# theovincent/iS-DQN

Hardware: AMD Instinct MI355X
Metric: gradient-steps/sec (batch=256, K=9, 84x84x4) (higher is better)
Workload: dtype bf16x3 (split-bf16 MFMA operands hi+lo, fp32 accumulate)

## Files before the change

### is-dqn_amd/csrc/conv_u8_pair.h

```cpp
#pragma once
#include "conv_img.h"

namespace isdqn {

constexpr int U8P_PB = 2;

template <int PASSES, int NSTEPS>
__global__ __launch_bounds__(GEMM_THREADS, 4) void conv_fwd_u8_pair_kernel(const ConvImgParams p) {
    ISDQN_EMPTY_KERNEL_RETURN
    constexpr int MT = 2, NT = 2, MTW = MT, NTHR = GEMM_THREADS, STACK_MAX = 4;
    using T = ConvImgTraits<MT, PASSES, true>;
    using GA = typename T::GA;
    extern __shared__ __attribute__((aligned(16))) char smem_raw[];
    __bf16* smem = reinterpret_cast<__bf16*>(smem_raw);
    __bf16* a_stage = smem;
    __bf16* img = smem + 2 * T::A_STAGE;
    const ConvGeom& g = p.g;
    const int tid = threadIdx.x, lane = tid & 63, wave = tid >> 6, grp = lane >> 4;
#if defined(ISDQN_DEV)
#define U8P_STAMP(i)                                                                                 \
    if (p.stamps != nullptr && threadIdx.x == 0) {                                                  \
        p.stamps[(int64_t)blockIdx.x * 8 + (i)] = (long long)__builtin_amdgcn_s_memtime();           \
        if ((i) == 0) p.stamps[(int64_t)blockIdx.x * 8 + 7] = (long long)__builtin_amdgcn_s_memrealtime(); \
    }
#else
#define U8P_STAMP(i)
#endif
    U8P_STAMP(0);
    const int T2 = p.tiles_per_img >> 1;
    int j, tp;
    xcd_image_tile((int)blockIdx.x, p.n_img, T2, j, tp);

    __shared__ __attribute__((aligned(16))) float s_par[3][64];
    float par_v = 0.f;
    {
        const int which = tid >> 6, ch = tid & 63;
        const float* src = which == 0 ? p.bias : which == 1 ? p.gamma : p.beta;
        const bool ok = tid < 192 && ch < g.cout_p && src != nullptr;
        ISDQN_BOUNDS_CHECK(ok ? src + ch : zero_chunk(), 4, 13);
        par_v = *(const ISDQN_GLOBAL float*)(ok ? src + ch : zero_chunk());
    }
    constexpr int nsteps = NSTEPS;
    const int k_last = g.K - 8;
    constexpr int A_PER = (GA::CHUNKS + NTHR - 1) / NTHR;
    int a_row[A_PER], a_var[A_PER], a_lds[A_PER];
    bool a_on[A_PER];
#pragma unroll
    for (int i = 0; i < A_PER; ++i) {
        int c = tid + i * NTHR;
        a_on[i] = c < GA::CHUNKS;
        if (!a_on[i]) c = 0;
        a_row[i] = stash_row(c);
        a_var[i] = (c & 3) * 8;
        a_lds[i] = a_row[i] * GA::PITCH + (c & 3) * 8;
    }
    constexpr int PF = 4;
    float sa[PF][A_PER][8];
    auto fetch = [&](int slot, int k) {
#pragma unroll
        for (int i = 0; i < A_PER; ++i) p.W.load(a_row[i], k + a_var[i], sa[slot][i]);
    };
    auto stash = [&](int slot, int stage) {
        __bf16* a_hi = a_stage + stage * T::A_STAGE;
        __bf16* a_lo = a_hi + GA::ELEMS;
#pragma unroll
        for (int i = 0; i < A_PER; ++i) {
            if (GA::CHUNKS % NTHR != 0 && !a_on[i]) continue;
            bf16x8 hi, lo;
            if constexpr (PASSES >= 2) {
                s8_unpack(sa[slot][i], hi, lo);
                *reinterpret_cast<bf16x8*>(a_lo + a_lds[i]) = lo;
            } else {
                s8_unpack_hi(sa[slot][i], hi);
            }
            *reinterpret_cast<bf16x8*>(a_hi + a_lds[i]) = hi;
        }
    };
    static_assert(NSTEPS >= PF + 2 && NSTEPS % 2 == 0, "ring of four slices + two staged ones");

    const FrameSrc& fs = p.fs;
    const uint8_t* base[STACK_MAX];
#pragma unroll
    for (int c = 0; c < STACK_MAX; ++c) {
        const int id = c < fs.stack ? fs.frame_id(j, c) : -1;
        base[c] = id >= 0 ? fs.frames + (int64_t)id * fs.stride : nullptr;
    }
    const uint8_t* zeros = reinterpret_cast<const uint8_t*>(zero_chunk());
    const int cpr = p.Wp / 8, per_plane = p.R * cpr, plane = p.R * p.Wp;
    unsigned long long raw[U8P_PB][STACK_MAX];
    auto request = [&](int row_base) {
#pragma unroll
        for (int k = 0; k < U8P_PB; ++k) {
            const int pos = k * NTHR + tid;
            const bool on = pos < per_plane;
            uint32_t lr, cx;
            p.d_chunk.divmod((uint32_t)(on ? pos : 0), lr, cx);
            const int iy = row_base + (int)lr, ix0 = (int)cx * 8 - g.pad;
            const bool ok = on && iy >= 0 && iy < fs.H && ix0 > -8 && ix0 < fs.W;
            const int ixc = min(max(ix0, 0), fs.W - 8);
            const int off = iy * fs.W + ixc;
#pragma unroll
            for (int c = 0; c < STACK_MAX; ++c) raw[k][c] = load_u64_unaligned((ok && base[c] != nullptr) ? base[c] + off : zeros);
        }
    };
    auto commit = [&]() {
#pragma unroll
        for (int k = 0; k < U8P_PB; ++k) {
            const int pos = k * NTHR + tid;
            const bool on = pos < per_plane;
            uint32_t lr, cx;
            p.d_chunk.divmod((uint32_t)(on ? pos : 0), lr, cx);
            const int ix0 = (int)cx * 8 - g.pad;
            const int sh = ix0 - min(max(ix0, 0), fs.W - 8);
            const int dst = (int)lr * p.Wp + (int)cx * 8;
#pragma unroll
            for (int c = 0; c < STACK_MAX; ++c) {
                if (c >= fs.stack) continue;
                float v[8];
                FrameSrc::patch8_cvt(raw[k][c], sh, v);
                bf16x8 hi;
                round8(v, hi);
                if (on) *reinterpret_cast<bf16x8*>(img + c * plane + dst) = hi;
            }
        }
    };
    auto tile_rows = [&](int tile) {
        const int oy_min = (int)g.d_wout.div((uint32_t)(tile * 128));
        return oy_min * g.stride - g.pad;
    };

    struct Frags {
        bf16x8 a_hi[MTW], a_lo[MTW], b_hi[NT];
    };

    auto do_tile = [&](auto it_c) {
        constexpr int it = decltype(it_c)::value;
        const int tile = 2 * tp + it;
        const int p0 = tile * 128;
        const int row_base = tile_rows(tile);
        const int full = (p.n_img / 8) * 8;
        const int old_wg8 = j < full ? (j >> 3) * p.tiles_per_img + tile : (j * p.tiles_per_img + tile) >> 3;
        const int rot = (int)((unsigned)old_wg8 % (unsigned)nsteps);
        auto slice = [&](int s) {
            const int k = s + rot;
            return k >= nsteps ? k - nsteps : k;
        };
#pragma unroll
        for (int d = 0; d < PF; ++d) fetch(d, slice(d) * GEMM_BK);
        if constexpr (it == 0) request(row_base);
        commit();
        U8P_STAMP(it == 0 ? 1 : 4);

        int b_org[NT], out_pix[NT];
#pragma unroll
        for (int nt = 0; nt < NT; ++nt) {
            int pp = p0 + wave * 32 + nt * 16 + (lane & 15);
            const bool in_img = pp < g.npix;
            pp = in_img ? pp : g.npix - 1;
            uint32_t oy_u, ox_u;
            g.d_wout.divmod((uint32_t)pp, oy_u, ox_u);
            const int oy = (int)oy_u, ox = (int)ox_u;
            out_pix[nt] = in_img ? oy * g.wout + ox : -1;
            const int ly0 = oy * g.stride - g.pad - row_base;
            const int lx0 = ox * g.stride;
            b_org[nt] = ly0 * p.Wp + lx0;
        }
        f32x4 acc[MTW][NT];
#pragma unroll
        for (int mt = 0; mt < MTW; ++mt)
#pragma unroll
            for (int nt = 0; nt < NT; ++nt) mfma_init(acc[mt][nt]);

        auto read_frags = [&](int stage, int kk, Frags& f) {
            const __bf16* a_hi = a_stage + stage * T::A_STAGE;
            const __bf16* a_lo = a_hi + GA::ELEMS;
#pragma unroll
            for (int mt = 0; mt < MTW; ++mt) {
                f.a_hi[mt] = read_frag<false, GA::PITCH>(a_hi, mt * 16, lane);
                if constexpr (PASSES >= 2) f.a_lo[mt] = read_frag<false, GA::PITCH>(a_lo, mt * 16, lane);
            }
            int kq = kk * GEMM_BK + grp * 8;
            kq = kq < k_last ? kq : k_last;
            const int c = kq >> 6, ky = (kq >> 3) & 7;
            const int tap_off = (c * p.R + ky) * p.Wp;
#pragma unroll
            for (int nt = 0; nt < NT; ++nt) {
                const __bf16* src = img + b_org[nt] + tap_off;
                typedef __attribute__((ext_vector_type(4))) __bf16 bf16x4;
                bf16x4 h0 = *reinterpret_cast<const bf16x4*>(src);
                bf16x4 h1 = *reinterpret_cast<const bf16x4*>(src + 4);
                f.b_hi[nt] = __builtin_shufflevector(h0, h1, 0, 1, 2, 3, 4, 5, 6, 7);
            }
        };
        auto mfma_step = [&](const Frags& f) {
#pragma unroll
            for (int nt = 0; nt < NT; ++nt)
#pragma unroll
                for (int mt = 0; mt < MTW; ++mt) {
                    if constexpr (PASSES >= 2) mfma_acc(acc[mt][nt], f.a_lo[mt], f.b_hi[nt]);
                    mfma_acc(acc[mt][nt], f.a_hi[mt], f.b_hi[nt]);
                }
        };
        Frags fr[2];
        if constexpr (it == 0) {
            if (tid < 192) s_par[tid >> 6][tid & 63] = par_v;
        }
        stash(0, 0);
        stash(1, 1);
        fetch(0, slice(PF) * GEMM_BK);
        fetch(1, slice(PF + 1) * GEMM_BK);
        __syncthreads();
        read_frags(0, slice(0), fr[0]);
        __syncthreads();
#pragma unroll
        for (int s = 0; s < NSTEPS; ++s) {
            if (s + 1 < NSTEPS) read_frags((s + 1) & 1, slice(s + 1), fr[(s + 1) & 1]);
            mfma_step(fr[s & 1]);
            if (s + 2 < NSTEPS) stash((s + 2) % PF, s & 1);
            if (s + 2 + PF < NSTEPS) fetch((s + 2) % PF, slice(s + 2 + PF) * GEMM_BK);
            if constexpr (it == 0) {
                if (s == NSTEPS - 3) request(tile_rows(tile + 1));
            }
            constexpr int N_MFMA = MTW * NT * (PASSES >= 3 ? 3 : PASSES);
#pragma unroll
            for (int i = 0; i < N_MFMA; ++i) {
                __builtin_amdgcn_sched_group_barrier(0x008, 1, 0);
                if (i < N_MFMA / 2) __builtin_amdgcn_sched_group_barrier(0x100, 1, 0);
                __builtin_amdgcn_sched_group_barrier(0x002, 2, 0);
            }
            __syncthreads();
        }

        U8P_STAMP(it == 0 ? 2 : 5);
        float bi[MTW][4], ga[MTW][4], be[MTW][4];
#pragma unroll
        for (int mt = 0; mt < MTW; ++mt) {
            const int ch0 = (mt * 16 + grp * 4) & 63;
            const float4 b4 = *reinterpret_cast<const float4*>(&s_par[0][ch0]);
            const float4 g4 = *reinterpret_cast<const float4*>(&s_par[1][ch0]);
            const float4 e4 = *reinterpret_cast<const float4*>(&s_par[2][ch0]);
            bi[mt][0] = b4.x; bi[mt][1] = b4.y; bi[mt][2] = b4.z; bi[mt][3] = b4.w;
            ga[mt][0] = g4.x; ga[mt][1] = g4.y; ga[mt][2] = g4.z; ga[mt][3] = g4.w;
            be[mt][0] = e4.x; be[mt][1] = e4.y; be[mt][2] = e4.z; be[mt][3] = e4.w;
        }
        const float inv_c = 1.0f / (float)g.cout;
        float zv[NT][MTW][4], s1[NT], s2[NT];
#pragma unroll
        for (int nt = 0; nt < NT; ++nt) {
            s1[nt] = s2[nt] = 0.f;
#pragma unroll
            for (int mt = 0; mt < MTW; ++mt)
#pragma unroll
                for (int r = 0; r < 4; ++r) {
                    int ch = mt * 16 + grp * 4 + r;
                    float zz = ch < g.cout ? acc[mt][nt][r] * p.scale + bi[mt][r] : 0.f;
                    zv[nt][mt][r] = zz;
                    s1[nt] += zz;
                    s2[nt] += zz * zz;
                }
            if (p.gamma != nullptr) {
                s1[nt] += __shfl_xor(s1[nt], 16); s1[nt] += __shfl_xor(s1[nt], 32);
                s2[nt] += __shfl_xor(s2[nt], 16); s2[nt] += __shfl_xor(s2[nt], 32);
            }
        }
#pragma unroll
        for (int nt = 0; nt < NT; ++nt) {
            float mean = 0.f, rstd = 1.f;
            if (p.gamma != nullptr) {
                mean = s1[nt] * inv_c;
                float var = fmaxf(s2[nt] * inv_c - mean * mean, 0.f);
                rstd = rsqrtf(var + 1e-6f);
            }
            if (out_pix[nt] >= 0) {
                const int64_t pix = (int64_t)j * g.npix + out_pix[nt];
#pragma unroll
                for (int mt = 0; mt < MTW; ++mt) {
                    int ch0 = mt * 16 + grp * 4;
                    if (ch0 >= g.cout_p) continue;
                    float4 a, zq;
                    float* ap = &a.x;
                    float* zp = &zq.x;
#pragma unroll
                    for (int r = 0; r < 4; ++r) {
                        float y = p.gamma != nullptr ? (zv[nt][mt][r] - mean) * (rstd * ga[mt][r]) + be[mt][r] : zv[nt][mt][r];
                        ap[r] = (ch0 + r < g.cout) ? fmaxf(y, 0.f) : 0.f;
                        zp[r] = zv[nt][mt][r];
                    }
                    s8_store_quad_paired(p.act + pix * g.cout_p, ch0, a.x, a.y, a.z, a.w);
                    if (j < p.z_img) *reinterpret_cast<float4*>(p.z + pix * g.cout_p + ch0) = zq;
                }
            }
        }
        U8P_STAMP(it == 0 ? 3 : 6);
    };
    do_tile(std::integral_constant<int, 0>{});
    do_tile(std::integral_constant<int, 1>{});
#undef U8P_STAMP
}

template <int PASSES, int NSTEPS>
static int launch_conv_fwd_u8_pair(const ConvImgParams& p, hipStream_t st) {
    using T = ConvImgTraits<2, PASSES, true>;
    const int lds = (2 * T::A_STAGE + T::B_PLANES * p.plane_elems) * 2;
    static LdsConfigured configured;
    if (int rc = ensure_dynamic_lds(&conv_fwd_u8_pair_kernel<PASSES, NSTEPS>, lds, configured)) return rc;
    const int grid = p.n_img * (p.tiles_per_img / 2);
    ISDQN_REPORT_OCCUPANCY((&conv_fwd_u8_pair_kernel<PASSES, NSTEPS>), GEMM_THREADS, lds, grid);
    hipLaunchKernelGGL((conv_fwd_u8_pair_kernel<PASSES, NSTEPS>), dim3(grid), dim3(GEMM_THREADS), lds, st, p);
    ISDQN_HIP_CHECK(hipGetLastError());
    return ISDQN_OK;
}

}
```

### is-dqn_amd/csrc/net_kernels.hip

```cpp
#include <stdarg.h>
#include <stdlib.h>

#include <algorithm>
#include <type_traits>
#include <vector>
#include <atomic>
#include <functional>

#include "conv_img.h"
#include "conv_u8_pair.h"
#include "conv_s8_pair.h"
#include "hl_gauss.h"
#include "net_plan.h"
#include "net_problems.h"

namespace isdqn {

__device__ inline double pow_int(double b, int t) {
    double r = 1.0, x = b;
    for (unsigned u = (unsigned)t; u != 0; u >>= 1) {
        if (u & 1u) r *= x;
        x *= x;
    }
    return r;
}


__global__ __launch_bounds__(256) void dense_post_kernel(const float* __restrict__ slabs, int n_slabs,
                                                         int64_t slab_stride, int64_t row_pitch, int rows, int F, int Fp,
                                                         const float* __restrict__ bias,
                                                         const float* __restrict__ gamma,
                                                         const float* __restrict__ beta, int has_relu,
                                                         float* __restrict__ act, float* __restrict__ z, int z_rows, int act_s8) {
    extern __shared__ float s_row[];
    __shared__ float s_red[2][4];
    const int row = blockIdx.x, tid = threadIdx.x;
    float* s_g = s_row + Fp;
    float* s_b = s_row + 2 * Fp;
    float s1 = 0.f, s2 = 0.f;
    for (int c = 2 * tid; c < Fp; c += 512) {
        float par[3][2];
#pragma unroll
        for (int w = 0; w < 3; ++w) {
            const float* src = w == 0 ? bias : w == 1 ? gamma : beta;
#pragma unroll
            for (int e = 0; e < 2; ++e)
            {
                ISDQN_BOUNDS_CHECK((src != nullptr && c + e < F) ? src + c + e : zero_chunk(), 4, 28);
                par[w][e] = *(const ISDQN_GLOBAL float*)((src != nullptr && c + e < F) ? src + c + e : zero_chunk());
            }
        }
        float v0 = 0.f, v1 = 0.f;
        const float* p = slabs + (int64_t)row * row_pitch + c;
        int s = 0;
        for (; s + 16 <= n_slabs; s += 16) {
            float2 t[16];
#pragma unroll
            for (int u = 0; u < 16; ++u) t[u] = *reinterpret_cast<const float2*>(p + (int64_t)(s + u) * slab_stride);
#pragma unroll
            for (int u = 0; u < 16; ++u) { v0 += t[u].x; v1 += t[u].y; }
        }
        if (s < n_slabs) {
            float2 t[16];
#pragma unroll
            for (int u = 0; u < 16; ++u)
                t[u] = *reinterpret_cast<const float2*>(p + (int64_t)min(s + u, n_slabs - 1) * slab_stride);
#pragma unroll
            for (int u = 0; u < 16; ++u) { v0 += (s + u < n_slabs) ? t[u].x : 0.f; v1 += (s + u < n_slabs) ? t[u].y : 0.f; }
        }
        v0 = c < F ? v0 + par[0][0] : 0.f;
        v1 = c + 1 < F ? v1 + par[0][1] : 0.f;
        s_row[c] = v0;
        s_row[c + 1] = v1;
        s_g[c] = par[1][0]; s_g[c + 1] = par[1][1];
        s_b[c] = par[2][0]; s_b[c + 1] = par[2][1];
        s1 += v0 + v1;
        s2 += v0 * v0 + v1 * v1;
    }
    float mean = 0.f, rstd = 1.f;
    if (gamma != nullptr) {
        for (int off = 32; off > 0; off >>= 1) {
            s1 += __shfl_xor(s1, off);
            s2 += __shfl_xor(s2, off);
        }
        if ((tid & 63) == 0) {
            s_red[0][tid >> 6] = s1;
            s_red[1][tid >> 6] = s2;
        }
        __syncthreads();
        s1 = s_red[0][0] + s_red[0][1] + s_red[0][2] + s_red[0][3];
        s2 = s_red[1][0] + s_red[1][1] + s_red[1][2] + s_red[1][3];
        mean = s1 / (float)F;
        float var = fmaxf(s2 / (float)F - mean * mean, 0.f);
// ... 987 lines not shown
    ConvGeom g;
    g.hin = l.hin; g.win = l.win; g.cin_p = l.cin_p; g.hout = l.hout; g.wout = l.wout;
    g.cout = l.cout; g.cout_p = l.cout_p; g.ksz = l.ksz; g.stride = l.stride; g.pad = l.pad;
    g.npix = l.npix; g.K = l.K;
    g.stride_sh = l.stride == 4 ? 2 : l.stride == 2 ? 1 : 0;
    g.d_npix = FastDiv(l.npix); g.d_wout = FastDiv(l.wout); g.d_cinp = FastDiv(l.cin_p);
    g.d_ksz = FastDiv(l.ksz); g.d_coutp = FastDiv(l.cout_p);
    return g;
}

constexpr int DZ_S8 = 1;

struct NetInput {
    const uint8_t* frames; int64_t frame_stride; const int* frame_ids; int paired_B;
    const float* obs; const float* obs2; int obs_split;
    int id_pitch = 0, id_off = 0;
};

template <int BM, int PASSES, bool U8>
static int launch_conv_fwd(const Layer& l, const float* params, const float* wmir, const NetInput& in, const float* act_in, int n_img,
                           int z_img, float* act, float* z, hipStream_t st) {
    ConvFwd<BM, PASSES, U8> p;
    p.g = conv_geom(l);
    p.W = MatSrc{wmir + l.w_off, l.K, l.cout_p, l.K, 1};
    p.in = act_in;
    p.fs = FrameSrc{in.frames, in.frame_stride, in.frame_ids, l.cin, in.paired_B, l.hin, l.win, in.id_pitch, in.id_off};
    p.bias = params + l.b_off;
    p.gamma = l.has_ln ? params + l.g_off : nullptr;
    p.beta = l.has_ln ? params + l.be_off : nullptr;
    p.scale = U8 ? (1.0f / 255.0f) : 1.0f;
    p.act = act; p.z = z;
    p.n_pix_total = n_img * l.npix;
    p.z_pix = z_img * l.npix;
    return launch_gemm(p, ceil_div(p.n_pix_total, 128), st);
}

static int conv_fwd_img(const Layer& l, bool x3, const float* params, const float* wmir, const NetInput& in, const float* act_in, int n_img,
                        int z_img, float* act, float* z, hipStream_t st, bool* done) {
    *done = false;
    if (act == nullptr || (z == nullptr && z_img > 0)) return ISDQN_OK;
    ConvImgParams ip;
    ip.g = conv_geom(l);
    const int mt = l.cout_p <= 32 ? 2 : 4;
    const int passes = x3 ? (l.is_u8 ? 2 : 3) : 1;
    ip.PP = l.is_u8 ? 0 : l.cin_p + (l.cin_p % 64 == 0 ? 16 : 8);
    int lds = conv_img_geometry(ip.g, l.is_u8, l.cin, passes >= 3 ? 2 : 1, mt, passes >= 2 ? 2 : 1, ip.R, ip.Wp,
                                ip.plane_elems, ip.PP);
    constexpr int LDS_LIMIT = 158 * 1024;
    if (lds > LDS_LIMIT || (l.is_u8 && (l.win < 8 || l.cin > 4))) return ISDQN_OK;
    if (!l.is_u8 && l.cin_p < 16) return ISDQN_OK;
    if (!l.is_u8 && l.npix <= 128) {
        const int want = ip.Wp + (((l.wout - ip.Wp) % 8) + 8) % 8;
        const int planes = passes >= 3 ? 2 : 1;
        const int lds2 = lds + planes * ip.R * (want - ip.Wp) * ip.PP * 2;
        const int stage2 = (passes >= 2 ? 2 : 1) * (mt * 16) * 48 * 2 * 2;
        const int old_total = lds > 80 * 1024 ? lds + stage2 : lds, new_total = lds2 > 80 * 1024 ? lds2 + stage2 : lds2;
        if (want != ip.Wp && new_total <= LDS_LIMIT && (old_total <= 80 * 1024) == (new_total <= 80 * 1024)) {
            ip.Wp = want;
            ip.plane_elems = ip.R * want * ip.PP;
            lds = lds2;
        }
    }
    ip.W = MatSrc{wmir + l.w_off, l.K, l.cout_p, l.K, 1};
    ip.in = act_in;
    ip.fs = FrameSrc{in.frames, in.frame_stride, in.frame_ids, l.cin, in.paired_B, l.hin, l.win, in.id_pitch, in.id_off};
    ip.bias = params + l.b_off;
    ip.gamma = l.has_ln ? params + l.g_off : nullptr;
    ip.beta = l.has_ln ? params + l.be_off : nullptr;
    ip.scale = l.is_u8 ? (1.0f / 255.0f) : 1.0f;
    ip.act = act; ip.z = z; ip.n_img = n_img; ip.z_img = z_img;
    ip.tiles_per_img = ceil_div(l.npix, 128);
    ip.d_chunk = FastDiv((uint32_t)(l.is_u8 ? ip.Wp / 8 : l.cin_p / 8));
    ip.d_Wp = FastDiv((uint32_t)ip.Wp);
    ip.d_R = FastDiv((uint32_t)ip.R);
    ip.order = PixelOrder(l.hout, l.wout, !l.is_u8 && ip.tiles_per_img == 1);
    ip.stamps = stamps_for(l.name);
    ip.ablate = 0;
#if defined(ISDQN_DEV)
    if (const char* e = getenv("ISDQN_ABLATE")) ip.ablate = atoi(e);
#endif
    *done = true;
    if (l.is_u8) {
#if !defined(ISDQN_NO_U8_PAIR)
        if (mt == 2 && ip.tiles_per_img % 2 == 0 && ip.R * (ip.Wp / 8) <= U8P_PB * GEMM_THREADS && l.cin == 4 && l.K == 256 && ip.ablate == 0)
            return passes == 2 ? launch_conv_fwd_u8_pair<2, 8>(ip, st) : launch_conv_fwd_u8_pair<1, 8>(ip, st);
#endif
        if (passes == 2) return mt == 2 ? launch_conv_fwd_img<2, 2, true>(ip, st) : launch_conv_fwd_img<4, 2, true>(ip, st);
        return mt == 2 ? launch_conv_fwd_img<2, 1, true>(ip, st) : launch_conv_fwd_img<4, 1, true>(ip, st);
    }
    const int stage_bytes = (passes >= 2 ? 2 : 1) * (mt * 16) * 48 * 2 * 2;
    static const bool no_kg = ISDQN_DEV_ENV("ISDQN_NO_KGROUPS");
    const bool kg2 = !no_kg && mt == 4 && lds > 80 * 1024 && lds + stage_bytes <= LDS_LIMIT &&
                     mt * 16 * 128 * 4 <= lds - stage_bytes && l.K >= 8 * GEMM_BK;
#if !defined(ISDQN_NO_U8_PAIR)
    if (passes == 3 && mt == 4 && kg2 && ip.tiles_per_img == 1 && l.K == 512 && n_img % 2 == 0 && ip.ablate == 0 && ip.stamps == nullptr &&
        ip.R * ip.Wp * (l.cin_p / 8) <= S8P_BATCH * GEMM_THREADS * 2)
        return launch_conv_fwd_s8_pair<8>(ip, st);
#endif
    if (passes == 3) return mt == 2 ? launch_conv_fwd_img<2, 3, false>(ip, st)
                          : kg2 ? launch_conv_fwd_img<4, 3, false, 2>(ip, st) : launch_conv_fwd_img<4, 3, false>(ip, st);
    return mt == 2 ? launch_conv_fwd_img<2, 1, false>(ip, st)
         : kg2 ? launch_conv_fwd_img<4, 1, false, 2>(ip, st) : launch_conv_fwd_img<4, 1, false>(ip, st);
}

static int conv_fwd(const Layer& l, bool x3, const float* params, const float* wmir, const NetInput& in, const float* act_in, int n_img,
                    int z_img, float* act, float* z, hipStream_t st) {
    bool done = false;
    int rc = conv_fwd_img(l, x3, params, wmir, in, act_in, n_img, z_img, act, z, st, &done);
    if (rc || done) return rc;
    const bool small = l.cout_p <= 32;
    if (l.is_u8) {
        if (x3) return small ? launch_conv_fwd<32, 2, true>(l, params, wmir, in, act_in, n_img, z_img, act, z, st)
                             : launch_conv_fwd<64, 2, true>(l, params, wmir, in, act_in, n_img, z_img, act, z, st);
        return small ? launch_conv_fwd<32, 1, true>(l, params, wmir, in, act_in, n_img, z_img, act, z, st)
                     : launch_conv_fwd<64, 1, true>(l, params, wmir, in, act_in, n_img, z_img, act, z, st);
    }
    if (x3) return small ? launch_conv_fwd<32, 3, false>(l, params, wmir, in, act_in, n_img, z_img, act, z, st)
                         : launch_conv_fwd<64, 3, false>(l, params, wmir, in, act_in, n_img, z_img, act, z, st);
    return small ? launch_conv_fwd<32, 1, false>(l, params, wmir, in, act_in, n_img, z_img, act, z, st)
                 : launch_conv_fwd<64, 1, false>(l, params, wmir, in, act_in, n_img, z_img, act, z, st);
}

template <int BM, int BN, int WM, int WN, bool ATR, bool BTR, int PASSES, bool AL, bool A2PART, bool ADAM = false, int S8M = 0>
static int launch_plain(const MatSrc& A, const float* A2, int a_split, const MatSrc& B, float* C, int ldc, int M,
                        int N, int K, int splits, int64_t slab_stride, hipStream_t st,
                        const AdamFuse* adam = nullptr) {
    PlainGemm<BM, BN, WM, WN, ATR, BTR, PASSES, AL, A2PART, ADAM, S8M> p;
    if (adam) p.adam = *adam;
    p.A = A; p.B = B; p.A2 = A2; p.a_split = a_split; p.C = C; p.ldc = ldc; p.M = M; p.N = N; p.K = K;
    p.tiles_m = ceil_div(M, BM); p.tiles_n = ceil_div(N, BN);
    int ksteps = ceil_div(K, GEMM_BK);
    if (splits < 1) splits = 1;
    if (splits > ksteps) splits = ksteps;
    p.steps_per_split = ceil_div(ksteps, splits);
    p.splits = ceil_div(ksteps, p.steps_per_split);
    p.slab_stride = slab_stride;
    return launch_gemm(p, p.tiles_m * p.tiles_n * p.splits, st);
}
static int effective_splits(int K, int splits) {
    int ksteps = ceil_div(K, GEMM_BK);
    if (splits < 1) splits = 1;
    if (splits > ksteps) splits = ksteps;
    int sps = ceil_div(ksteps, splits);
    return ceil_div(ksteps, sps);
}

template <bool ATR, bool BTR, bool AL = true, bool A2PART = false, int S8M = 0>
static int plain_big(bool x3, const MatSrc& A, const float* A2, int a_split, const MatSrc& B, float* C, int ldc,
                     int M, int N, int K, int splits, int64_t slab_stride, hipStream_t st) {
    if (x3)
        return launch_plain<128, 128, 2, 2, ATR, BTR, 3, AL, A2PART, false, S8M>(A, A2, a_split, B, C, ldc, M, N, K, splits,
                                                                                 slab_stride, st);
    return launch_plain<128, 128, 2, 2, ATR, BTR, 1, AL, A2PART, false, S8M>(A, A2, a_split, B, C, ldc, M, N, K, splits,
                                                                             slab_stride, st);
}

template <bool ATR, bool BTR, int S8M = 0>
static int plain_narrow(bool x3, const MatSrc& A, const MatSrc& B, float* C, int ldc, int M, int N, int K, int splits,
                        int64_t slab_stride, hipStream_t st) {
    if (x3) return launch_plain<128, 64, 2, 2, ATR, BTR, 3, true, false, false, S8M>(A, nullptr, 0, B, C, ldc, M, N, K, splits, slab_stride, st);
    return launch_plain<128, 64, 2, 2, ATR, BTR, 1, true, false, false, S8M>(A, nullptr, 0, B, C, ldc, M, N, K, splits, slab_stride, st);
}

static int dense_fwd(const Layer& l, bool x3, const float* params, const float* wmir, const NetInput& in, const float* act_in, int rows,
                     int z_rows, float* slab, float* act, float* z, hipStream_t st, bool skip_post = false) {
    MatSrc A, B;
    const float* A2 = nullptr;
    int a_split = 0;
// ... 1172 lines not shown
```

Baseline: 4172.

## Replace paired u8 conv kernel with persistent kernel keeping weights resident in LDS

Swaps the two-tile-per-block u8 first-layer conv for a persistent kernel with a grid sized to the CU count. Each workgroup loads the full 32xK weight slab into LDS once and then loops over many image tiles, prefetching the next item's frames while the current one computes. This removes the per-tile weight refetch, the staged-slice ring and the per-step barriers. In exchange it uses more LDS per block, allows only 2 workgroups per CU, and relies on the persistent loop hiding frame-load latency.

```diff
diff --git a/is-dqn_amd/csrc/conv_u8_pair.h b/is-dqn_amd/csrc/conv_u8_pair.h
--- a/is-dqn_amd/csrc/conv_u8_pair.h
+++ /dev/null
@@ -1,314 +0,0 @@
-#pragma once
-#include "conv_img.h"
-
-namespace isdqn {
-
-constexpr int U8P_PB = 2;
-
-template <int PASSES, int NSTEPS>
-__global__ __launch_bounds__(GEMM_THREADS, 4) void conv_fwd_u8_pair_kernel(const ConvImgParams p) {
-    ISDQN_EMPTY_KERNEL_RETURN
-    constexpr int MT = 2, NT = 2, MTW = MT, NTHR = GEMM_THREADS, STACK_MAX = 4;
-    using T = ConvImgTraits<MT, PASSES, true>;
-    using GA = typename T::GA;
-    extern __shared__ __attribute__((aligned(16))) char smem_raw[];
-    __bf16* smem = reinterpret_cast<__bf16*>(smem_raw);
-    __bf16* a_stage = smem;
-    __bf16* img = smem + 2 * T::A_STAGE;
-    const ConvGeom& g = p.g;
-    const int tid = threadIdx.x, lane = tid & 63, wave = tid >> 6, grp = lane >> 4;
-#if defined(ISDQN_DEV)
-#define U8P_STAMP(i)                                                                                 \
-    if (p.stamps != nullptr && threadIdx.x == 0) {                                                  \
-        p.stamps[(int64_t)blockIdx.x * 8 + (i)] = (long long)__builtin_amdgcn_s_memtime();           \
-        if ((i) == 0) p.stamps[(int64_t)blockIdx.x * 8 + 7] = (long long)__builtin_amdgcn_s_memrealtime(); \
-    }
-#else
-#define U8P_STAMP(i)
-#endif
-    U8P_STAMP(0);
-    const int T2 = p.tiles_per_img >> 1;
-    int j, tp;
-    xcd_image_tile((int)blockIdx.x, p.n_img, T2, j, tp);
-
-    __shared__ __attribute__((aligned(16))) float s_par[3][64];
-    float par_v = 0.f;
-    {
-        const int which = tid >> 6, ch = tid & 63;
-        const float* src = which == 0 ? p.bias : which == 1 ? p.gamma : p.beta;
-        const bool ok = tid < 192 && ch < g.cout_p && src != nullptr;
-        ISDQN_BOUNDS_CHECK(ok ? src + ch : zero_chunk(), 4, 13);
-        par_v = *(const ISDQN_GLOBAL float*)(ok ? src + ch : zero_chunk());
-    }
-    constexpr int nsteps = NSTEPS;
-    const int k_last = g.K - 8;
-    constexpr int A_PER = (GA::CHUNKS + NTHR - 1) / NTHR;
-    int a_row[A_PER], a_var[A_PER], a_lds[A_PER];
-    bool a_on[A_PER];
-#pragma unroll
-    for (int i = 0; i < A_PER; ++i) {
-        int c = tid + i * NTHR;
-        a_on[i] = c < GA::CHUNKS;
-        if (!a_on[i]) c = 0;
-        a_row[i] = stash_row(c);
-        a_var[i] = (c & 3) * 8;
-        a_lds[i] = a_row[i] * GA::PITCH + (c & 3) * 8;
-    }
-    constexpr int PF = 4;
-    float sa[PF][A_PER][8];
-    auto fetch = [&](int slot, int k) {
-#pragma unroll
-        for (int i = 0; i < A_PER; ++i) p.W.load(a_row[i], k + a_var[i], sa[slot][i]);
-    };
-    auto stash = [&](int slot, int stage) {
-        __bf16* a_hi = a_stage + stage * T::A_STAGE;
-        __bf16* a_lo = a_hi + GA::ELEMS;
-#pragma unroll
-        for (int i = 0; i < A_PER; ++i) {
-            if (GA::CHUNKS % NTHR != 0 && !a_on[i]) continue;
-            bf16x8 hi, lo;
-            if constexpr (PASSES >= 2) {
-                s8_unpack(sa[slot][i], hi, lo);
-                *reinterpret_cast<bf16x8*>(a_lo + a_lds[i]) = lo;
-            } else {
-                s8_unpack_hi(sa[slot][i], hi);
-            }
-            *reinterpret_cast<bf16x8*>(a_hi + a_lds[i]) = hi;
-        }
-    };
-    static_assert(NSTEPS >= PF + 2 && NSTEPS % 2 == 0, "ring of four slices + two staged ones");
-
-    const FrameSrc& fs = p.fs;
-    const uint8_t* base[STACK_MAX];
-#pragma unroll
-    for (int c = 0; c < STACK_MAX; ++c) {
-        const int id = c < fs.stack ? fs.frame_id(j, c) : -1;
-        base[c] = id >= 0 ? fs.frames + (int64_t)id * fs.stride : nullptr;
-    }
-    const uint8_t* zeros = reinterpret_cast<const uint8_t*>(zero_chunk());
-    const int cpr = p.Wp / 8, per_plane = p.R * cpr, plane = p.R * p.Wp;
-    unsigned long long raw[U8P_PB][STACK_MAX];
-    auto request = [&](int row_base) {
-#pragma unroll
-        for (int k = 0; k < U8P_PB; ++k) {
-            const int pos = k * NTHR + tid;
-            const bool on = pos < per_plane;
-            uint32_t lr, cx;
-            p.d_chunk.divmod((uint32_t)(on ? pos : 0), lr, cx);
-            const int iy = row_base + (int)lr, ix0 = (int)cx * 8 - g.pad;
-            const bool ok = on && iy >= 0 && iy < fs.H && ix0 > -8 && ix0 < fs.W;
-            const int ixc = min(max(ix0, 0), fs.W - 8);
-            const int off = iy * fs.W + ixc;
-#pragma unroll
-            for (int c = 0; c < STACK_MAX; ++c) raw[k][c] = load_u64_unaligned((ok && base[c] != nullptr) ? base[c] + off : zeros);
-        }
-    };
-    auto commit = [&]() {
-#pragma unroll
-        for (int k = 0; k < U8P_PB; ++k) {
-            const int pos = k * NTHR + tid;
-            const bool on = pos < per_plane;
-            uint32_t lr, cx;
-            p.d_chunk.divmod((uint32_t)(on ? pos : 0), lr, cx);
-            const int ix0 = (int)cx * 8 - g.pad;
-            const int sh = ix0 - min(max(ix0, 0), fs.W - 8);
-            const int dst = (int)lr * p.Wp + (int)cx * 8;
-#pragma unroll
-            for (int c = 0; c < STACK_MAX; ++c) {
-                if (c >= fs.stack) continue;
-                float v[8];
-                FrameSrc::patch8_cvt(raw[k][c], sh, v);
-                bf16x8 hi;
-                round8(v, hi);
-                if (on) *reinterpret_cast<bf16x8*>(img + c * plane + dst) = hi;
-            }
-        }
-    };
-    auto tile_rows = [&](int tile) {
-        const int oy_min = (int)g.d_wout.div((uint32_t)(tile * 128));
-        return oy_min * g.stride - g.pad;
-    };
-
-    struct Frags {
-        bf16x8 a_hi[MTW], a_lo[MTW], b_hi[NT];
-    };
-
-    auto do_tile = [&](auto it_c) {
-        constexpr int it = decltype(it_c)::value;
-        const int tile = 2 * tp + it;
-        const int p0 = tile * 128;
-        const int row_base = tile_rows(tile);
-        const int full = (p.n_img / 8) * 8;
-        const int old_wg8 = j < full ? (j >> 3) * p.tiles_per_img + tile : (j * p.tiles_per_img + tile) >> 3;
-        const int rot = (int)((unsigned)old_wg8 % (unsigned)nsteps);
-        auto slice = [&](int s) {
-            const int k = s + rot;
-            return k >= nsteps ? k - nsteps : k;
-        };
-#pragma unroll
-        for (int d = 0; d < PF; ++d) fetch(d, slice(d) * GEMM_BK);
-        if constexpr (it == 0) request(row_base);
-        commit();
-        U8P_STAMP(it == 0 ? 1 : 4);
-
-        int b_org[NT], out_pix[NT];
-#pragma unroll
-        for (int nt = 0; nt < NT; ++nt) {
-            int pp = p0 + wave * 32 + nt * 16 + (lane & 15);
-            const bool in_img = pp < g.npix;
-            pp = in_img ? pp : g.npix - 1;
-            uint32_t oy_u, ox_u;
-            g.d_wout.divmod((uint32_t)pp, oy_u, ox_u);
-            const int oy = (int)oy_u, ox = (int)ox_u;
-            out_pix[nt] = in_img ? oy * g.wout + ox : -1;
-            const int ly0 = oy * g.stride - g.pad - row_base;
-            const int lx0 = ox * g.stride;
-            b_org[nt] = ly0 * p.Wp + lx0;
-        }
-        f32x4 acc[MTW][NT];
-#pragma unroll
-        for (int mt = 0; mt < MTW; ++mt)
-#pragma unroll
-            for (int nt = 0; nt < NT; ++nt) mfma_init(acc[mt][nt]);
-
-        auto read_frags = [&](int stage, int kk, Frags& f) {
-            const __bf16* a_hi = a_stage + stage * T::A_STAGE;
-            const __bf16* a_lo = a_hi + GA::ELEMS;
-#pragma unroll
-            for (int mt = 0; mt < MTW; ++mt) {
-                f.a_hi[mt] = read_frag<false, GA::PITCH>(a_hi, mt * 16, lane);
-                if constexpr (PASSES >= 2) f.a_lo[mt] = read_frag<false, GA::PITCH>(a_lo, mt * 16, lane);
-            }
-            int kq = kk * GEMM_BK + grp * 8;
-            kq = kq < k_last ? kq : k_last;
-            const int c = kq >> 6, ky = (kq >> 3) & 7;
-            const int tap_off = (c * p.R + ky) * p.Wp;
-#pragma unroll
-            for (int nt = 0; nt < NT; ++nt) {
-                const __bf16* src = img + b_org[nt] + tap_off;
-                typedef __attribute__((ext_vector_type(4))) __bf16 bf16x4;
-                bf16x4 h0 = *reinterpret_cast<const bf16x4*>(src);
-                bf16x4 h1 = *reinterpret_cast<const bf16x4*>(src + 4);
-                f.b_hi[nt] = __builtin_shufflevector(h0, h1, 0, 1, 2, 3, 4, 5, 6, 7);
-            }
-        };
-        auto mfma_step = [&](const Frags& f) {
-#pragma unroll
-            for (int nt = 0; nt < NT; ++nt)
-#pragma unroll
-                for (int mt = 0; mt < MTW; ++mt) {
-                    if constexpr (PASSES >= 2) mfma_acc(acc[mt][nt], f.a_lo[mt], f.b_hi[nt]);
-                    mfma_acc(acc[mt][nt], f.a_hi[mt], f.b_hi[nt]);
-                }
-        };
-        Frags fr[2];
-        if constexpr (it == 0) {
-            if (tid < 192) s_par[tid >> 6][tid & 63] = par_v;
-        }
-        stash(0, 0);
-        stash(1, 1);
-        fetch(0, slice(PF) * GEMM_BK);
-        fetch(1, slice(PF + 1) * GEMM_BK);
-        __syncthreads();
-        read_frags(0, slice(0), fr[0]);
-        __syncthreads();
-#pragma unroll
-        for (int s = 0; s < NSTEPS; ++s) {
-            if (s + 1 < NSTEPS) read_frags((s + 1) & 1, slice(s + 1), fr[(s + 1) & 1]);
-            mfma_step(fr[s & 1]);
-            if (s + 2 < NSTEPS) stash((s + 2) % PF, s & 1);
-            if (s + 2 + PF < NSTEPS) fetch((s + 2) % PF, slice(s + 2 + PF) * GEMM_BK);
-            if constexpr (it == 0) {
-                if (s == NSTEPS - 3) request(tile_rows(tile + 1));
-            }
-            constexpr int N_MFMA = MTW * NT * (PASSES >= 3 ? 3 : PASSES);
-#pragma unroll
-            for (int i = 0; i < N_MFMA; ++i) {
-                __builtin_amdgcn_sched_group_barrier(0x008, 1, 0);
-                if (i < N_MFMA / 2) __builtin_amdgcn_sched_group_barrier(0x100, 1, 0);
-                __builtin_amdgcn_sched_group_barrier(0x002, 2, 0);
-            }
-            __syncthreads();
-        }
-
-        U8P_STAMP(it == 0 ? 2 : 5);
-        float bi[MTW][4], ga[MTW][4], be[MTW][4];
-#pragma unroll
-        for (int mt = 0; mt < MTW; ++mt) {
-            const int ch0 = (mt * 16 + grp * 4) & 63;
-            const float4 b4 = *reinterpret_cast<const float4*>(&s_par[0][ch0]);
-            const float4 g4 = *reinterpret_cast<const float4*>(&s_par[1][ch0]);
-            const float4 e4 = *reinterpret_cast<const float4*>(&s_par[2][ch0]);
-            bi[mt][0] = b4.x; bi[mt][1] = b4.y; bi[mt][2] = b4.z; bi[mt][3] = b4.w;
-            ga[mt][0] = g4.x; ga[mt][1] = g4.y; ga[mt][2] = g4.z; ga[mt][3] = g4.w;
-            be[mt][0] = e4.x; be[mt][1] = e4.y; be[mt][2] = e4.z; be[mt][3] = e4.w;
-        }
-        const float inv_c = 1.0f / (float)g.cout;
-        float zv[NT][MTW][4], s1[NT], s2[NT];
-#pragma unroll
-        for (int nt = 0; nt < NT; ++nt) {
-            s1[nt] = s2[nt] = 0.f;
-#pragma unroll
-            for (int mt = 0; mt < MTW; ++mt)
-#pragma unroll
-                for (int r = 0; r < 4; ++r) {
-                    int ch = mt * 16 + grp * 4 + r;
-                    float zz = ch < g.cout ? acc[mt][nt][r] * p.scale + bi[mt][r] : 0.f;
-                    zv[nt][mt][r] = zz;
-                    s1[nt] += zz;
-                    s2[nt] += zz * zz;
-                }
-            if (p.gamma != nullptr) {
-                s1[nt] += __shfl_xor(s1[nt], 16); s1[nt] += __shfl_xor(s1[nt], 32);
-                s2[nt] += __shfl_xor(s2[nt], 16); s2[nt] += __shfl_xor(s2[nt], 32);
-            }
-        }
-#pragma unroll
-        for (int nt = 0; nt < NT; ++nt) {
-            float mean = 0.f, rstd = 1.f;
-            if (p.gamma != nullptr) {
-                mean = s1[nt] * inv_c;
-                float var = fmaxf(s2[nt] * inv_c - mean * mean, 0.f);
-                rstd = rsqrtf(var + 1e-6f);
-            }
-            if (out_pix[nt] >= 0) {
-                const int64_t pix = (int64_t)j * g.npix + out_pix[nt];
-#pragma unroll
-                for (int mt = 0; mt < MTW; ++mt) {
-                    int ch0 = mt * 16 + grp * 4;
-                    if (ch0 >= g.cout_p) continue;
-                    float4 a, zq;
-                    float* ap = &a.x;
-                    float* zp = &zq.x;
-#pragma unroll
-                    for (int r = 0; r < 4; ++r) {
-                        float y = p.gamma != nullptr ? (zv[nt][mt][r] - mean) * (rstd * ga[mt][r]) + be[mt][r] : zv[nt][mt][r];
-                        ap[r] = (ch0 + r < g.cout) ? fmaxf(y, 0.f) : 0.f;
-                        zp[r] = zv[nt][mt][r];
-                    }
-                    s8_store_quad_paired(p.act + pix * g.cout_p, ch0, a.x, a.y, a.z, a.w);
-                    if (j < p.z_img) *reinterpret_cast<float4*>(p.z + pix * g.cout_p + ch0) = zq;
-                }
-            }
-        }
-        U8P_STAMP(it == 0 ? 3 : 6);
-    };
-    do_tile(std::integral_constant<int, 0>{});
-    do_tile(std::integral_constant<int, 1>{});
-#undef U8P_STAMP
-}
-
-template <int PASSES, int NSTEPS>
-static int launch_conv_fwd_u8_pair(const ConvImgParams& p, hipStream_t st) {
-    using T = ConvImgTraits<2, PASSES, true>;
-    const int lds = (2 * T::A_STAGE + T::B_PLANES * p.plane_elems) * 2;
-    static LdsConfigured configured;
-    if (int rc = ensure_dynamic_lds(&conv_fwd_u8_pair_kernel<PASSES, NSTEPS>, lds, configured)) return rc;
-    const int grid = p.n_img * (p.tiles_per_img / 2);
-    ISDQN_REPORT_OCCUPANCY((&conv_fwd_u8_pair_kernel<PASSES, NSTEPS>), GEMM_THREADS, lds, grid);
-    hipLaunchKernelGGL((conv_fwd_u8_pair_kernel<PASSES, NSTEPS>), dim3(grid), dim3(GEMM_THREADS), lds, st, p);
-    ISDQN_HIP_CHECK(hipGetLastError());
-    return ISDQN_OK;
-}
-
-}
diff --git a/is-dqn_amd/csrc/conv_u8_persistent.h b/is-dqn_amd/csrc/conv_u8_persistent.h
--- /dev/null
+++ b/is-dqn_amd/csrc/conv_u8_persistent.h
@@ -0,0 +1,350 @@
+#pragma once
+#include "conv_img.h"
+
+namespace isdqn {
+
+constexpr int U8W_PB = 2;
+constexpr int U8W_MAX_ITEMS = 64;
+constexpr int U8W_WG_PER_CU = 2;
+
+template <int NSTEPS>
+struct U8wGeom {
+    static constexpr int PITCH = NSTEPS * GEMM_BK + 16;
+    static constexpr int ELEMS = 32 * PITCH;
+    static_assert(((2 * PITCH) / 16) % 4 == 2, "ds_read_b128 conflict-free pitch rule (ConvImgTraits)");
+};
+
+template <int PASSES, int NSTEPS>
+__global__ __launch_bounds__(GEMM_THREADS, 2) void conv_fwd_u8_persistent_kernel(const ConvImgParams p) {
+    ISDQN_EMPTY_KERNEL_RETURN
+    constexpr int MT = 2, NT = 2, MTW = MT, NTHR = GEMM_THREADS, STACK_MAX = 4;
+    constexpr int A_PLANES = PASSES >= 2 ? 2 : 1;
+    using WG = U8wGeom<NSTEPS>;
+    extern __shared__ __attribute__((aligned(16))) char smem_raw[];
+    __bf16* w_hi = reinterpret_cast<__bf16*>(smem_raw);
+    __bf16* w_lo = w_hi + WG::ELEMS;
+    __bf16* img = w_hi + A_PLANES * WG::ELEMS;
+    __shared__ __attribute__((aligned(16))) float s_par[3][64];
+    __shared__ int s_ids[U8W_MAX_ITEMS][STACK_MAX];
+    const ConvGeom& g = p.g;
+    const int tid = threadIdx.x, lane = tid & 63, wave = tid >> 6, grp = lane >> 4;
+    const int n_work = p.n_img * p.tiles_per_img, grid = (int)gridDim.x, w0 = (int)blockIdx.x;
+    const int n_items = (n_work - 1 - w0) / grid + 1;
+#if defined(ISDQN_DEV)
+#define U8W_STAMP(w, i)                                                                              \
+    if (p.stamps != nullptr && threadIdx.x == 0) {                                                  \
+        p.stamps[(int64_t)(w) * 8 + (i)] = (long long)__builtin_amdgcn_s_memtime();                  \
+        if ((i) == 0) p.stamps[(int64_t)(w) * 8 + 7] = (long long)__builtin_amdgcn_s_memrealtime(); \
+        if ((i) == 4) p.stamps[(int64_t)(w) * 8 + 5] = p.stamps[(int64_t)(w) * 8 + 4];              \
+    }
+#else
+#define U8W_STAMP(w, i)
+#endif
+    U8W_STAMP(w0, 0);
+
+    float par_v = 0.f;
+    {
+        const int which = tid >> 6, ch = tid & 63;
+        const float* src = which == 0 ? p.bias : which == 1 ? p.gamma : p.beta;
+        const bool ok = tid < 192 && ch < g.cout_p && src != nullptr;
+        ISDQN_BOUNDS_CHECK(ok ? src + ch : zero_chunk(), 4, 13);
+        par_v = *(const ISDQN_GLOBAL float*)(ok ? src + ch : zero_chunk());
+    }
+    constexpr int W_CPR = NSTEPS * GEMM_BK / 8;
+    constexpr int W_PER = 32 * W_CPR / NTHR;
+    static_assert((32 * W_CPR) % NTHR == 0, "whole weight chunks per thread");
+    float wv[W_PER][8];
+#pragma unroll
+    for (int i = 0; i < W_PER; ++i) {
+        const int c = tid + i * NTHR;
+        p.W.load(c / W_CPR, (c % W_CPR) * 8, wv[i]);
+    }
+    const FrameSrc& fs = p.fs;
+    int my_id = -1;
+    {
+        const int i = tid >> 2, c = tid & 3;
+        if (i < n_items && c < fs.stack) {
+            int j, tile;
+            xcd_image_tile(w0 + i * grid, p.n_img, p.tiles_per_img, j, tile);
+            my_id = fs.frame_id(j, c);
+        }
+    }
+
+    const uint8_t* zeros = reinterpret_cast<const uint8_t*>(zero_chunk());
+    const int cpr = p.Wp / 8, per_plane = p.R * cpr, plane = p.R * p.Wp;
+    unsigned long long raw[U8W_PB][STACK_MAX];
+    auto tile_rows = [&](int tile) {
+        const int oy_min = (int)g.d_wout.div((uint32_t)(tile * 128));
+        return oy_min * g.stride - g.pad;
+    };
+    auto request = [&](const uint8_t* const (&base)[STACK_MAX], int row_base) {
+#pragma unroll
+        for (int k = 0; k < U8W_PB; ++k) {
+            const int pos = k * NTHR + tid;
+            const bool on = pos < per_plane;
+            uint32_t lr, cx;
+            p.d_chunk.divmod((uint32_t)(on ? pos : 0), lr, cx);
+            const int iy = row_base + (int)lr, ix0 = (int)cx * 8 - g.pad;
+            const bool ok = on && iy >= 0 && iy < fs.H && ix0 > -8 && ix0 < fs.W;
+            const int ixc = min(max(ix0, 0), fs.W - 8);
+            const int off = iy * fs.W + ixc;
+#pragma unroll
+            for (int c = 0; c < STACK_MAX; ++c) raw[k][c] = load_u64_unaligned((ok && base[c] != nullptr) ? base[c] + off : zeros);
+        }
+    };
+    auto request_item = [&](int i, const int (&ids)[STACK_MAX]) {
+        int j, tile;
+        xcd_image_tile(w0 + i * grid, p.n_img, p.tiles_per_img, j, tile);
+        const uint8_t* base[STACK_MAX];
+#pragma unroll
+        for (int c = 0; c < STACK_MAX; ++c) base[c] = ids[c] >= 0 ? fs.frames + (int64_t)ids[c] * fs.stride : nullptr;
+        request(base, tile_rows(tile));
+    };
+    auto commit = [&]() {
+#pragma unroll
+        for (int k = 0; k < U8W_PB; ++k) {
+            const int pos = k * NTHR + tid;
+            const bool on = pos < per_plane;
+            uint32_t lr, cx;
+            p.d_chunk.divmod((uint32_t)(on ? pos : 0), lr, cx);
+            const int ix0 = (int)cx * 8 - g.pad;
+            const int sh = ix0 - min(max(ix0, 0), fs.W - 8);
+            const int dst = (int)lr * p.Wp + (int)cx * 8;
+#pragma unroll
+            for (int c = 0; c < STACK_MAX; ++c) {
+                if (c >= fs.stack) continue;
+                float v[8];
+                FrameSrc::patch8_cvt(raw[k][c], sh, v);
+                bf16x8 hi;
+                round8(v, hi);
+                if (on) *reinterpret_cast<bf16x8*>(img + c * plane + dst) = hi;
+            }
+        }
+    };
+
+    {
+        int j, tile;
+        xcd_image_tile(w0, p.n_img, p.tiles_per_img, j, tile);
+        int ids[STACK_MAX];
+#pragma unroll
+        for (int c = 0; c < STACK_MAX; ++c) ids[c] = c < fs.stack ? fs.frame_id(j, c) : -1;
+        request_item(0, ids);
+    }
+#pragma unroll
+    for (int i = 0; i < W_PER; ++i) {
+        const int c = tid + i * NTHR;
+        const int dst = (c / W_CPR) * WG::PITCH + (c % W_CPR) * 8;
+        bf16x8 hi, lo;
+        if constexpr (PASSES >= 2) {
+            s8_unpack(wv[i], hi, lo);
+            *reinterpret_cast<bf16x8*>(w_lo + dst) = lo;
+        } else {
+            s8_unpack_hi(wv[i], hi);
+        }
+        *reinterpret_cast<bf16x8*>(w_hi + dst) = hi;
+    }
+    if (tid < 192) s_par[tid >> 6][tid & 63] = par_v;
+    s_ids[tid >> 2][tid & 3] = my_id;
+    commit();
+    __syncthreads();
+    auto item_ids = [&](int i, int (&ids)[STACK_MAX]) {
+#pragma unroll
+        for (int c = 0; c < STACK_MAX; ++c) ids[c] = s_ids[i][c];
+    };
+    if (n_items > 1) {
+        int ids[STACK_MAX];
+        item_ids(1, ids);
+        request_item(1, ids);
+    }
+
+    struct Frags {
+        bf16x8 a_hi[MTW], a_lo[MTW], b_hi[NT];
+    };
+    constexpr int nsteps = NSTEPS;
+    const int k_last = g.K - 8;
+    const int full = (p.n_img / 8) * 8;
+    for (int it = 0; it < n_items; ++it) {
+        const int w = w0 + it * grid;
+        int j, tile;
+        xcd_image_tile(w, p.n_img, p.tiles_per_img, j, tile);
+        if (it > 0) {
+            U8W_STAMP(w, 0);
+            __syncthreads();
+        }
+        U8W_STAMP(w, 1);
+        const int p0 = tile * 128;
+        const int row_base = tile_rows(tile);
+        const int old_wg8 = j < full ? (j >> 3) * p.tiles_per_img + tile : (j * p.tiles_per_img + tile) >> 3;
+        const int rot = (int)((unsigned)old_wg8 % (unsigned)nsteps);
+        auto slice = [&](int s) {
+            const int k = s + rot;
+            return k >= nsteps ? k - nsteps : k;
+        };
+
+        int b_org[NT], out_pix[NT];
+#pragma unroll
+        for (int nt = 0; nt < NT; ++nt) {
+            int pp = p0 + wave * 32 + nt * 16 + (lane & 15);
+            const bool in_img = pp < g.npix;
+            pp = in_img ? pp : g.npix - 1;
+            uint32_t oy_u, ox_u;
+            g.d_wout.divmod((uint32_t)pp, oy_u, ox_u);
+            const int oy = (int)oy_u, ox = (int)ox_u;
+            out_pix[nt] = in_img ? oy * g.wout + ox : -1;
+            const int ly0 = oy * g.stride - g.pad - row_base;
+            const int lx0 = ox * g.stride;
+            b_org[nt] = ly0 * p.Wp + lx0;
+        }
+        f32x4 acc[MTW][NT];
+#pragma unroll
+        for (int mt = 0; mt < MTW; ++mt)
+#pragma unroll
+            for (int nt = 0; nt < NT; ++nt) mfma_init(acc[mt][nt]);
+
+        auto read_frags = [&](int kk, Frags& f) {
+#pragma unroll
+            for (int mt = 0; mt < MTW; ++mt) {
+                f.a_hi[mt] = read_frag<false, WG::PITCH>(w_hi + kk * GEMM_BK, mt * 16, lane);
+                if constexpr (PASSES >= 2) f.a_lo[mt] = read_frag<false, WG::PITCH>(w_lo + kk * GEMM_BK, mt * 16, lane);
+            }
+            int kq = kk * GEMM_BK + grp * 8;
+            kq = kq < k_last ? kq : k_last;
+            const int c = kq >> 6, ky = (kq >> 3) & 7;
+            const int tap_off = (c * p.R + ky) * p.Wp;
+#pragma unroll
+            for (int nt = 0; nt < NT; ++nt) {
+                const __bf16* src = img + b_org[nt] + tap_off;
+                typedef __attribute__((ext_vector_type(4))) __bf16 bf16x4;
+                bf16x4 h0 = *reinterpret_cast<const bf16x4*>(src);
+                bf16x4 h1 = *reinterpret_cast<const bf16x4*>(src + 4);
+                f.b_hi[nt] = __builtin_shufflevector(h0, h1, 0, 1, 2, 3, 4, 5, 6, 7);
+            }
+        };
+        auto mfma_step = [&](const Frags& f) {
+#pragma unroll
+            for (int nt = 0; nt < NT; ++nt)
+#pragma unroll
+                for (int mt = 0; mt < MTW; ++mt) {
+                    if constexpr (PASSES >= 2) mfma_acc(acc[mt][nt], f.a_lo[mt], f.b_hi[nt]);
+                    mfma_acc(acc[mt][nt], f.a_hi[mt], f.b_hi[nt]);
+                }
+        };
+        Frags fr[2];
+        read_frags(slice(0), fr[0]);
+#pragma unroll
+        for (int s = 0; s < NSTEPS; ++s) {
+            if (s + 1 < NSTEPS) read_frags(slice(s + 1), fr[(s + 1) & 1]);
+            mfma_step(fr[s & 1]);
+        }
+        __syncthreads();
+        U8W_STAMP(w, 2);
+        if (it + 1 < n_items) {
+            commit();
+            if (it + 2 < n_items) {
+                int ids[STACK_MAX];
+                item_ids(it + 2, ids);
+                request_item(it + 2, ids);
+            }
+        }
+        U8W_STAMP(w, 3);
+
+        float bi[MTW][4], ga[MTW][4], be[MTW][4];
+#pragma unroll
+        for (int mt = 0; mt < MTW; ++mt) {
+            const int ch0 = (mt * 16 + grp * 4) & 63;
+            const float4 b4 = *reinterpret_cast<const float4*>(&s_par[0][ch0]);
+            const float4 g4 = *reinterpret_cast<const float4*>(&s_par[1][ch0]);
+            const float4 e4 = *reinterpret_cast<const float4*>(&s_par[2][ch0]);
+            bi[mt][0] = b4.x; bi[mt][1] = b4.y; bi[mt][2] = b4.z; bi[mt][3] = b4.w;
+            ga[mt][0] = g4.x; ga[mt][1] = g4.y; ga[mt][2] = g4.z; ga[mt][3] = g4.w;
+            be[mt][0] = e4.x; be[mt][1] = e4.y; be[mt][2] = e4.z; be[mt][3] = e4.w;
+        }
+        const float inv_c = 1.0f / (float)g.cout;
+        float zv[NT][MTW][4], s1[NT], s2[NT];
+#pragma unroll
+        for (int nt = 0; nt < NT; ++nt) {
+            s1[nt] = s2[nt] = 0.f;
+#pragma unroll
+            for (int mt = 0; mt < MTW; ++mt)
+#pragma unroll
+                for (int r = 0; r < 4; ++r) {
+                    int ch = mt * 16 + grp * 4 + r;
+                    float zz = ch < g.cout ? acc[mt][nt][r] * p.scale + bi[mt][r] : 0.f;
+                    zv[nt][mt][r] = zz;
+                    s1[nt] += zz;
+                    s2[nt] += zz * zz;
+                }
+            if (p.gamma != nullptr) {
+                s1[nt] += __shfl_xor(s1[nt], 16); s1[nt] += __shfl_xor(s1[nt], 32);
+                s2[nt] += __shfl_xor(s2[nt], 16); s2[nt] += __shfl_xor(s2[nt], 32);
+            }
+        }
+#pragma unroll
+        for (int nt = 0; nt < NT; ++nt) {
+            float mean = 0.f, rstd = 1.f;
+            if (p.gamma != nullptr) {
+                mean = s1[nt] * inv_c;
+                float var = fmaxf(s2[nt] * inv_c - mean * mean, 0.f);
+                rstd = rsqrtf(var + 1e-6f);
+            }
+            if (out_pix[nt] >= 0) {
+                const int64_t pix = (int64_t)j * g.npix + out_pix[nt];
+#pragma unroll
+                for (int mt = 0; mt < MTW; ++mt) {
+                    int ch0 = mt * 16 + grp * 4;
+                    if (ch0 >= g.cout_p) continue;
+                    float4 a, zq;
+                    float* ap = &a.x;
+                    float* zp = &zq.x;
+#pragma unroll
+                    for (int r = 0; r < 4; ++r) {
+                        float y = p.gamma != nullptr ? (zv[nt][mt][r] - mean) * (rstd * ga[mt][r]) + be[mt][r] : zv[nt][mt][r];
+                        ap[r] = (ch0 + r < g.cout) ? fmaxf(y, 0.f) : 0.f;
+                        zp[r] = zv[nt][mt][r];
+                    }
+                    s8_store_quad_paired(p.act + pix * g.cout_p, ch0, a.x, a.y, a.z, a.w);
+                    if (j < p.z_img) *reinterpret_cast<float4*>(p.z + pix * g.cout_p + ch0) = zq;
+                }
+            }
+        }
+        U8W_STAMP(w, 4);
+    }
+#undef U8W_STAMP
+}
+
+static inline int u8w_grid(int n_work) {
+    static int cus[ISDQN_MAX_DEVICES] = {0};
+    const int d = current_device_slot();
+    if (cus[d] == 0) {
+        int dev = 0, n = 0;
+        if (hipGetDevice(&dev) != hipSuccess || hipDeviceGetAttribute(&n, hipDeviceAttributeMultiprocessorCount, dev) != hipSuccess || n <= 0)
+            n = 256;
+        cus[d] = n;
+    }
+    int per_cu = U8W_WG_PER_CU;
+#if defined(ISDQN_DEV)
+    if (const char* e = getenv("ISDQN_U8W_PER_CU")) per_cu = atoi(e) > 0 ? atoi(e) : per_cu;
+#endif
+    int grid = (cus[d] * per_cu) / 8 * 8;
+    grid = std::max(grid, round_up(ceil_div(n_work, U8W_MAX_ITEMS), 8));
+    return std::max(1, std::min(grid, n_work));
+}
+
+template <int NSTEPS>
+static inline int u8w_lds_bytes(int passes, int plane_elems) {
+    return ((passes >= 2 ? 2 : 1) * U8wGeom<NSTEPS>::ELEMS + plane_elems) * 2;
+}
+
+template <int PASSES, int NSTEPS>
+static int launch_conv_fwd_u8_persistent(const ConvImgParams& p, hipStream_t st) {
+    const int lds = u8w_lds_bytes<NSTEPS>(PASSES, p.plane_elems);
+    static LdsConfigured configured;
+    if (int rc = ensure_dynamic_lds(&conv_fwd_u8_persistent_kernel<PASSES, NSTEPS>, lds, configured)) return rc;
+    const int grid = u8w_grid(p.n_img * p.tiles_per_img);
+    ISDQN_REPORT_OCCUPANCY((&conv_fwd_u8_persistent_kernel<PASSES, NSTEPS>), GEMM_THREADS, lds, grid);
+    hipLaunchKernelGGL((conv_fwd_u8_persistent_kernel<PASSES, NSTEPS>), dim3(grid), dim3(GEMM_THREADS), lds, st, p);
+    ISDQN_HIP_CHECK(hipGetLastError());
+    return ISDQN_OK;
+}
+
+}
diff --git a/is-dqn_amd/csrc/net_kernels.hip b/is-dqn_amd/csrc/net_kernels.hip
--- a/is-dqn_amd/csrc/net_kernels.hip
+++ b/is-dqn_amd/csrc/net_kernels.hip
@@ -8,7 +8,7 @@
 #include <functional>
 
 #include "conv_img.h"
-#include "conv_u8_pair.h"
+#include "conv_u8_persistent.h"
 #include "conv_s8_pair.h"
 #include "hl_gauss.h"
 #include "net_plan.h"
@@ -1162,8 +1162,9 @@
     *done = true;
     if (l.is_u8) {
 #if !defined(ISDQN_NO_U8_PAIR)
-        if (mt == 2 && ip.tiles_per_img % 2 == 0 && ip.R * (ip.Wp / 8) <= U8P_PB * GEMM_THREADS && l.cin == 4 && l.K == 256 && ip.ablate == 0)
-            return passes == 2 ? launch_conv_fwd_u8_pair<2, 8>(ip, st) : launch_conv_fwd_u8_pair<1, 8>(ip, st);
+        if (mt == 2 && ip.R * (ip.Wp / 8) <= U8W_PB * GEMM_THREADS && l.cin == 4 && l.K == 256 && ip.ablate == 0 &&
+            u8w_lds_bytes<8>(passes, ip.plane_elems) <= LDS_LIMIT)
+            return passes == 2 ? launch_conv_fwd_u8_persistent<2, 8>(ip, st) : launch_conv_fwd_u8_persistent<1, 8>(ip, st);
 #endif
         if (passes == 2) return mt == 2 ? launch_conv_fwd_img<2, 2, true>(ip, st) : launch_conv_fwd_img<4, 2, true>(ip, st);
         return mt == 2 ? launch_conv_fwd_img<2, 1, true>(ip, st) : launch_conv_fwd_img<4, 1, true>(ip, st);
```

After: 4184 (median of 6 runs). No clear change (+0.3%).
